# zdzhaoyong/GSLAM

Measured on AMD Instinct MI355X. Metric: orb_extract_plus_bf_match_Mkeypoints_per_s, higher is better.
Workload: dtype u8

## Files before the change

### gslam_amd/csrc/orb.hip

```cpp
#include <stdlib.h>

#include "common.h"
#include "orb_quadtree.h"
#include "../../include/gslam_orb_tables.h"

namespace {

constexpr int kEdge = GH_ORB_EDGE;
constexpr int kCell = GH_ORB_CELL;
constexpr int kCap = GH_ORB_CELL_CAP;
constexpr int kMaxL = GH_ORB_MAX_LEVELS;
constexpr int kHistBins = kCap * 256;
constexpr int kCellRec = 8;

enum {
  kDbgCells = 0,
  kDbgDenseCells,
  kDbgOverflowCells,
  kDbgCapCells,
  kDbgRankDropped,
  kDbgStrongSilenced,
  kDbgMaxQueue,
  kDbgMaxNz,
  kDbgSelCut,
// ... 14 lines not shown
};

__device__ __forceinline__ int xcd_strip_tile(int lin, int total) {
  const int chunk = (total + 7) >> 3;
  return (lin & 7) * chunk + (lin >> 3);
}

__global__ void copy_rows_kernel(const uint8_t* __restrict__ src, size_t src_frame_stride, int src_pitch,
                                 uint8_t* __restrict__ dst, size_t dst_frame_stride, int dst_pitch, int w, int h) {
  int x = blockIdx.x * blockDim.x + threadIdx.x;
  int y = blockIdx.y;
  if (x >= w) return;
  dst[(size_t)blockIdx.z * dst_frame_stride + (size_t)y * dst_pitch + x] =
      src[(size_t)blockIdx.z * src_frame_stride + (size_t)y * src_pitch + x];
}

constexpr int kResizeRows = 4;
constexpr int kResizeCols = 8;

typedef uint32_t u32x4_a4 __attribute__((ext_vector_type(4), aligned(4)));

__device__ __forceinline__ uint32_t mad_u24(uint32_t a, uint32_t b, uint32_t c) {
  uint32_t d;
  asm("v_mad_u32_u24 %0, %1, %2, %3" : "=v"(d) : "v"(a), "v"(b), "v"(c));
  return d;
}

struct ResizeTabs {
  const uint32_t* xtab;
  const uint32_t* xsel;
  const uint32_t* xwgt;
  const uint32_t* ytab;
  const uint32_t* mtab = nullptr;
  const uint32_t* mcw = nullptr;
};

__device__ __forceinline__ void resize_item(const LevelView& src, const uint8_t* __restrict__ s, uint8_t* __restrict__ d,
                                            int dst_pitch, const ResizeTabs& tb, int x8, int y0, int y_end, bool guard_frame) {
  typedef unsigned short u16x2 __attribute__((ext_vector_type(2)));
  const int sx0 = (int)(tb.xtab[x8] >> 16);
  const uint32_t al = (uint32_t)(sx0 & 3);
  const uint32_t d0 = (uint32_t)sx0 & ~3u;
  const uint4 sa = *reinterpret_cast<const uint4*>(tb.xsel + x8), sb = *reinterpret_cast<const uint4*>(tb.xsel + x8 + 4);
  const uint4 wa = *reinterpret_cast<const uint4*>(tb.xwgt + x8), wb = *reinterpret_cast<const uint4*>(tb.xwgt + x8 + 4);
  const uint32_t selp[8] = {sa.x, sa.y, sa.z, sa.w, sb.x, sb.y, sb.z, sb.w};
  const uint32_t wx[8] = {wa.x, wa.y, wa.z, wa.w, wb.x, wb.y, wb.z, wb.w};
  const bool guard = guard_frame && (int)d0 + 16 > src.pitch;
  const uint32_t last_dw = (uint32_t)src.pitch - 4u;
  const uint32_t pitch = (uint32_t)src.pitch;
#pragma unroll
  for (int rr = 0; rr < kResizeRows; ++rr) {
    const int y = y0 + rr;
    if (y >= y_end) break;
    const uint32_t ty = tb.ytab[y];
    const uint32_t sy = ty >> 16;
    const uint32_t fy = ty & 0xFFFFu;
    const uint32_t sy1 = sy + 1 < (uint32_t)src.h ? sy + 1 : (uint32_t)src.h - 1;
    const uint32_t o0 = __umul24(sy, pitch), o1 = __umul24(sy1, pitch);
    u32x4_a4 u, v;
    if (guard && sy1 == (uint32_t)src.h - 1) {
      auto ld = [&](uint32_t row, uint32_t k) { return *reinterpret_cast<const uint32_t*>(s + row + min(d0 + 4u * k, last_dw)); };
      u = u32x4_a4{ld(o0, 0), ld(o0, 1), ld(o0, 2), ld(o0, 3)};
      v = u32x4_a4{ld(o1, 0), ld(o1, 1), ld(o1, 2), ld(o1, 3)};
    } else {
      u = *reinterpret_cast<const u32x4_a4*>(s + (o0 + d0));
      v = *reinterpret_cast<const u32x4_a4*>(s + (o1 + d0));
    }
    const uint32_t uw[3] = {__builtin_amdgcn_alignbyte(u.y, u.x, al), __builtin_amdgcn_alignbyte(u.z, u.y, al),
                            __builtin_amdgcn_alignbyte(u.w, u.z, al)};
    const uint32_t vw[3] = {__builtin_amdgcn_alignbyte(v.y, v.x, al), __builtin_amdgcn_alignbyte(v.z, v.y, al),
                            __builtin_amdgcn_alignbyte(v.w, v.z, al)};
    const uint32_t wy0 = 4u * (2048u - fy), wy1 = 4u * fy;
    uint32_t r[8];
#pragma unroll
    for (int i = 0; i < 8; ++i) {
      const int wsel = i >= 4 ? 1 : 0;
      const u16x2 pu = __builtin_bit_cast(u16x2, __builtin_amdgcn_perm(uw[wsel + 1], uw[wsel], selp[i]));
      const u16x2 pv = __builtin_bit_cast(u16x2, __builtin_amdgcn_perm(vw[wsel + 1], vw[wsel], selp[i]));
      const u16x2 w2 = __builtin_bit_cast(u16x2, wx[i]);
      const uint32_t h0 = __builtin_amdgcn_udot2(pu, w2, 0u, false);
      const uint32_t h1 = __builtin_amdgcn_udot2(pv, w2, 0u, false);
      r[i] = mad_u24(h0, wy0, mad_u24(h1, wy1, 1u << 23));
    }
    uint2 packed;
    packed.x = __builtin_amdgcn_perm(__builtin_amdgcn_perm(r[3], r[2], 0x0c0c0703u), __builtin_amdgcn_perm(r[1], r[0], 0x0c0c0703u), 0x05040100u);
    packed.y = __builtin_amdgcn_perm(__builtin_amdgcn_perm(r[7], r[6], 0x0c0c0703u), __builtin_amdgcn_perm(r[5], r[4], 0x0c0c0703u), 0x05040100u);
    *reinterpret_cast<uint2*>(d + (__umul24((uint32_t)y, (uint32_t)dst_pitch) + (uint32_t)x8)) = packed;
  }
}

__global__ __launch_bounds__(256) void resize_kernel(LevelView src, uint8_t* __restrict__ dst_base,
                                                     size_t dst_frame_stride, int dst_pitch, int wd, int hd,
                                                     ResizeTabs tb, int groups_per_row,
                                                     uint32_t groups_inv, int n_items, int tail_unsafe_frame) {
  const int item = blockIdx.x * 256 + threadIdx.x;
  if (item >= n_items) return;
  const int rg = (int)__umulhi((uint32_t)item, groups_inv);
  const int x8 = (item - rg * groups_per_row) * kResizeCols;
  const int y0 = rg * kResizeRows;
  resize_item(src, src.base + (size_t)blockIdx.y * src.frame_stride, dst_base + (size_t)blockIdx.y * dst_frame_stride, dst_pitch,
              tb, x8, y0, min(hd, y0 + kResizeRows), (int)blockIdx.y == tail_unsafe_frame);
}

struct NextLevel {
  uint8_t* dst_base;
  size_t dst_frame_stride;
  int dst_pitch, hd;
  ResizeTabs tb;
  const int32_t* gx0;
  const int32_t* gy0;
  int tail_unsafe_frame;
  uint32_t tiles_inv = 0, nbx_inv = 0;
  uint8_t* plane = nullptr;
  size_t plane_frame_stride = 0;
  int plane_pitch = 0;
};

inline uint32_t magic_div(uint32_t d, uint32_t n_max) {
  if (d == 0) return 0;
  if (d == 1) return 0;
  const uint64_t inv = ((1ull << 32) + d - 1) / d;
  const uint64_t excess = inv * d - (1ull << 32);
  return (inv < (1ull << 32) && (uint64_t)n_max * excess < (1ull << 32)) ? (uint32_t)inv : 0u;
}

struct ResizeOps {
  uint4 aw[4];
  int cwv[4];
  uint32_t ty;
};
__device__ __forceinline__ ResizeOps resize_tile_mfma_load(int ax, const ResizeTabs& tb, int g0, int ng, int r0, int r1) {
  const int lane = threadIdx.x & 63, n16 = lane & 15;
  const int rb = __builtin_amdgcn_readfirstlane((int)(threadIdx.x >> 6));
  const int ncb = (ng + 1) >> 1;
  const int yq = r0 + 16 * rb + n16, y = yq < r1 ? yq : r1 - 1;
  ResizeOps o;
  o.ty = tb.ytab[y];
#pragma unroll
  for (int cb = 0; cb < 4; ++cb) {
    const int g = g0 + 2 * (cb < ncb ? cb : 0);
    o.aw[cb] = *reinterpret_cast<const uint4*>(tb.mtab + ((size_t)g * 64 + lane) * 4);
    o.cwv[cb] = (int)tb.mcw[g] - ax;
  }
  return o;
}
__device__ __forceinline__ void resize_tile_mfma(const uint8_t* tile, int tile_pitch, int oy, uint8_t* __restrict__ d,
                                                 int dst_pitch, const ResizeOps& ops, int g0, int ng, int r0, int r1,
                                                 uint32_t* __restrict__ dbg) {
  typedef _Float16 f16x8 __attribute__((ext_vector_type(8)));
  typedef float f32x4 __attribute__((ext_vector_type(4)));
  const int lane = threadIdx.x & 63, n16 = lane & 15, q4 = lane >> 4;
  const int rb = __builtin_amdgcn_readfirstlane((int)(threadIdx.x >> 6));
  if (r0 + 16 * rb >= r1) return;
  const int ncb = (ng + 1) >> 1;
  const int yq = r0 + 16 * rb + n16, y = yq < r1 ? yq : r1 - 1;
  const uint32_t ty = ops.ty;
  const uint4 (&aw)[4] = ops.aw;
  const int (&cwv)[4] = ops.cwv;
  const int R = (int)(ty >> 16) - oy;
  const uint32_t fy = ty & 0xFFFFu;
  const uint32_t wy0 = 2048u - fy, wy1 = fy, c23 = 1u << 23, k64 = 0x64646464u;
  const uint8_t* row1 = tile + R * tile_pitch + 8 * q4;
  const uint8_t* row2 = row1 + tile_pitch;
  const uint32_t rowoff = __umul24((uint32_t)y, (uint32_t)dst_pitch);
#pragma unroll
  for (int half = 0; half < 2; ++half) {
    if (2 * half >= ncb) break;
    uint32_t u[2][4], v[2][4];
#pragma unroll
    for (int e = 0; e < 2; ++e) {
      const int cb = 2 * half + e;
      const uint2 b1 = *reinterpret_cast<const uint2*>(row1 + cwv[cb]);
      const uint2 b2 = *reinterpret_cast<const uint2*>(row2 + cwv[cb]);
      uint4 f1, f2;
      f1.x = __builtin_amdgcn_perm(k64, b1.x, 0x04010400u);
// ... 129 lines not shown
  uint32_t a, d;
  __device__ __forceinline__ explicit CompassQ(uint32_t t) : a((((t + 1u) >> 2) + 127u) * 0x01010101u), d((128u - ((t + 1u) >> 2)) * 0x01010101u) {}
};
__device__ __forceinline__ uint32_t fast_compass4_q(const CompassQ& k, uint32_t wc, uint32_t wl, uint32_t wr, uint32_t wu, uint32_t wd) {
  constexpr uint32_t kQ = 0x3F3F3F3Fu;
  const uint32_t c = (wc >> 2) & kQ, u = (wu >> 2) & kQ, d = (wd >> 2) & kQ;
  const uint32_t l = (__builtin_amdgcn_alignbyte(wc, wl, 1) >> 2) & kQ, r = (__builtin_amdgcn_alignbyte(wr, wc, 3) >> 2) & kQ;
  const uint32_t A = c + k.a, Dk = c + k.d;
  const uint32_t not_bright_lr = (A - l) & (A - r);
  const uint32_t bright = __builtin_amdgcn_bitop3_b32(A - u, A - d, not_bright_lr, 0x15);
  const uint32_t dark_lr = (Dk - l) | (Dk - r);
  const uint32_t dark = __builtin_amdgcn_bitop3_b32(Dk - u, Dk - d, dark_lr, 0xA8);
  return bright | dark;
}

#ifndef GH_FAST_WAVES
#define GH_FAST_WAVES 8
#endif
#ifdef GH_ORB_PHASES
__device__ unsigned int* g_orb_phase_buf;
__shared__ unsigned long long ph_t;
__shared__ unsigned int ph_slot;
#define GH_PHASE_START() do { if (threadIdx.x == 0) ph_t = wall_clock64(); } while (0)
#define GH_PHASE(k) do { if (threadIdx.x == 0) { const unsigned long long now_ = wall_clock64(); g_orb_phase_buf[(size_t)ph_slot * 8 + (k)] = (unsigned int)(now_ - ph_t); ph_t = now_; } } while (0)
#else
#define GH_PHASE_START()
#define GH_PHASE(k)
#endif
constexpr int kTileW = 96;
constexpr int kTileH = 72;
constexpr int kScoreH = 66;
constexpr int kScoreOff = 3;

__device__ __forceinline__ void fast_tile_coords(const NextLevel& nx, int nbx, int nby, int tile_id, int& frame, int& bx, int& by) {
  if (nx.tiles_inv != 0u && nx.nbx_inv != 0u) {
    frame = (int)__umulhi((uint32_t)tile_id, nx.tiles_inv);
    const int trem = tile_id - frame * (nbx * nby);
    by = (int)__umulhi((uint32_t)trem, nx.nbx_inv);
    bx = trem - by * nbx;
  } else {
    frame = tile_id / (nbx * nby);
    const int trem = tile_id - frame * (nbx * nby);
    bx = trem % nbx;
    by = trem / nbx;
  }
}
__device__ __forceinline__ const uint4* fast_tile_src(const LevelView& lv, int frame, int bx, int by, int i) {
  const int row = (int)(__umul24((uint32_t)i, 10923u) >> 16), c = i - row * 6;
  int gy = kEdge + 64 * by - 4 + row;
  gy = gy < 0 ? 0 : (gy > lv.h - 1 ? lv.h - 1 : gy);
  int gx = 64 * bx + 16 * c;
  gx = gx > lv.pitch - 16 ? lv.pitch - 16 : gx;
  return reinterpret_cast<const uint4*>(lv.base + (size_t)frame * lv.frame_stride + (__umul24((uint32_t)gy, (uint32_t)lv.pitch) + (uint32_t)gx));
}

constexpr uint32_t kWeakCell = 0xFFFFFFFFu;

__device__ __forceinline__ int hint_threshold(uint32_t word, uint32_t epoch, int ini_th) {
  return ((word >> 16) & 255u) != 0u && (epoch & 1u) != 0u ? ini_th : (int)(word & 255u);
}

template <int PITCH, bool WEAK>
__device__ __forceinline__ int fast_cell_stage(const uint8_t* sc, uint16_t* list2, uint32_t* list, int lane, int ini_th,
                                               uint32_t* __restrict__ rec, uint32_t* __restrict__ ovf,
                                               uint32_t* __restrict__ dbg, int* nz_out) {
  static_assert(PITCH % 4 == 0, "a lane reads its 16 score bytes as dwords");
  const uint64_t lt_mask = (1ull << lane) - 1ull;
  int nz = 0;
  {
    const int row = lane >> 1, cb = 16 * (lane & 1);
    const uint32_t* sp32 = reinterpret_cast<const uint32_t*>(&sc[row * PITCH + cb]);
    uint32_t nzb = 0;
#pragma unroll
    for (int dwi = 0; dwi < 4; ++dwi) {
      const uint32_t w = sp32[dwi];
      const uint32_t f = ((((w & 0x7f7f7f7fu) + 0x7f7f7f7fu) | w) >> 7) & 0x01010101u;
      nzb |= __builtin_amdgcn_udot4(f, 0x08040201u, 0u, false) << (4 * dwi);
    }
    const int cnt = __popc(nzb);
    const int incl = wave_incl_scan_i32(cnt);
// ... 72 lines not shown
        int m2 = 0;
        for (int base = 0; base < n; base += 64) {
          const int i = base + lane;
          const uint32_t e = i < n ? list[i] : 0u;
          const bool keep = i < n && (int)(e >> 10) > ini_th;
          const uint64_t m = __ballot(keep);
          if (keep) list[m2 + __popcll(m & lt_mask)] = e;
          m2 += __popcll(m);
        }
        if (dbg != nullptr && lane == 0 && m2 != n) atomicAdd(&dbg[kDbgStrongSilenced], 1u);
        n = m2;
      }
      if (dbg != nullptr && lane == 0 && !strong && n > 0) atomicAdd(&dbg[kDbgWeakCells], 1u);
    }
    if (dbg != nullptr && lane == 0) {
      atomicAdd(&dbg[kDbgDenseCells], 1u);
      if (n > kCap) atomicAdd(&dbg[kDbgRankDropped], 1u);
    }
    for (int base = 0; base < n; base += 64) {
      const int i = base + lane;
      const uint32_t key = i < n ? list[i] : 0xFFFFFFFFu;
      int rank = 0;
      for (int j = 0; j < n; ++j) rank += list[j] > key ? 1 : 0;
      const bool keep = i < n && rank < kCap;
      const uint64_t m = __ballot(keep);
      if (keep) put_entry(kept + __popcll(m & lt_mask), ((uint32_t)rank << 18) | (key ^ 0x3FFu));
      kept += __popcll(m);
    }
  }
  return kept;
}

template <bool PLANE, bool TWO_PHASE>
__device__ __forceinline__ void fast_cells_tile(const LevelView& lv, int ncx, int ncy, int min_th, int ini_th, bool two,
                                                const uint32_t* __restrict__ hint, int th_a, uint32_t epoch,
                                                uint32_t* __restrict__ cell_cnt, uint32_t* __restrict__ cell_ent,
                                                int cells_per_frame, int cell_off, int n_frames, const NextLevel& nx,
                                                uint32_t* __restrict__ dbg, int tile_id) {
  bool phase_a = TWO_PHASE && two;
  int score_th = min_th;
  constexpr int kScoreW = 68;
  constexpr int kScoreBytes = kScoreH * kScoreW + 8;
  constexpr int kQueueLen = kScoreH * kScoreW;
  __shared__ __attribute__((aligned(16))) uint8_t tile[kTileH * kTileW];
  __shared__ __attribute__((aligned(16))) uint8_t score[kScoreBytes];
  uint32_t(*lists)[256] = reinterpret_cast<uint32_t(*)[256]>(tile);
  static_assert(sizeof(tile) >= 4 * 256 * sizeof(uint32_t), "four 1 KB lists fit the tile");
  __shared__ uint16_t queue[kQueueLen];
  __shared__ int q_count;
  __shared__ uint16_t bit_pos[32];
  GH_PHASE_START();

  const int tid = threadIdx.x;
  __builtin_assume(tid >= 0 && tid < 256);
  const int nbx = (ncx + 1) >> 1, nby = (ncy + 1) >> 1;
  int frame, bx, by;
  fast_tile_coords(nx, nbx, nby, tile_id, frame, bx, by);
  if constexpr (TWO_PHASE) {
    if (phase_a) {
      if (hint != nullptr) th_a = hint_threshold(hint[__builtin_amdgcn_readfirstlane(frame) * kMaxL], epoch, ini_th);
      score_th = th_a;
    }
  }
  const bool pass1_quant = TWO_PHASE && phase_a && th_a > ini_th;
#ifdef GH_ORB_PHASES
  if (threadIdx.x == 0) {
    const unsigned int slot_ = (unsigned int)(frame * cells_per_frame + cell_off + by * nbx + bx);
    ph_slot = slot_;
    g_orb_phase_buf[(size_t)slot_ * 8 + 6] = 1u;
  }
#endif
  static_assert(kTileW / 16 == 6 && kTileH * (kTileW / 16) <= 512 && kTileH * (kTileW / 16) > 256, "two 16-byte items per thread");
  if (tid == 0) q_count = 0;
  const int x0 = kEdge + 64 * bx, y0 = kEdge + 64 * by;
  const int oy = y0 - 4;
  const int ax = 64 * bx;
  const uint8_t* img = lv.base + (size_t)frame * lv.frame_stride;

  bool resized = false;
  ResizeOps rops;
  int rg0 = 0, rng = 0, rr0 = 0, rr1 = 0;
  if (nx.dst_base != nullptr && nx.tb.mtab != nullptr && by > 0 && by < nby - 1 && bx < nbx - 1) {
    rg0 = nx.gx0[bx];
    rng = nx.gx0[bx + 1] - rg0;
    if (rng <= 8) {
      rr0 = nx.gy0[by];
      rr1 = nx.gy0[by + 1];
      rops = resize_tile_mfma_load(ax, nx.tb, rg0, rng, rr0, rr1);
      resized = true;
    }
  }
  for (int i = tid; i < kTileH * (kTileW / 16); i += 256) *reinterpret_cast<uint4*>(&tile[16 * i]) = *fast_tile_src(lv, frame, bx, by, i);
  if (tid < 32) {
    const int ix = tid ^ 15;
    const int k = pass1_quant ? tid >> 3 : (ix & 1) + 2 * (ix >> 4), trip = pass1_quant ? 7 - (tid & 7) : (ix >> 1) & 7;
    bit_pos[tid] = (uint16_t)(1024 * trip + 1 + k);
  }
  __syncthreads();
  GH_PHASE(0);
  if (resized) resize_tile_mfma(tile, kTileW, oy, nx.dst_base + (size_t)frame * nx.dst_frame_stride, nx.dst_pitch, rops, rg0, rng, rr0, rr1, dbg);

  static_assert(kScoreBytes % 16 == 0, "the score tile is cleared by 16-byte stores");
  for (int i = tid; i < kScoreBytes / 16; i += 256) reinterpret_cast<uint4*>(score)[i] = make_uint4(0u, 0u, 0u, 0u);
  const int sx_lo = max(0, kEdge - (x0 - 1)), sx_hi = min(kScoreH, lv.w - kEdge - (x0 - 1));
  const bool interior = sx_lo == 0 && sx_hi == kScoreH && y0 - 1 >= kEdge && y0 - 1 + kScoreH <= lv.h - kEdge;
  constexpr int kItemsPerRow = 17, kItems = kScoreH * kItemsPerRow;
  constexpr int kTrips = (kItems + 255) / 256;
  static_assert(2 * kTrips <= 14 && kScoreW == 4 * kItemsPerRow, "candidate bits of all trips share one dword");
  const uint32_t* tile32 = reinterpret_cast<const uint32_t*>(tile);
  auto pass1 = [&](int th, bool quant) {
    const uint32_t t = (uint32_t)__builtin_amdgcn_readfirstlane(min(max(th, 0), 255));
    const uint32_t tid3856 = (uint32_t)tid * 3856u;
    uint32_t allbits = 0;
    auto trips = [&](auto flags4, int shift, uint32_t mask) {
#pragma unroll
      for (int trip = 0; trip < kTrips; ++trip) {
        const int item = 256 * trip + tid;
        if (item < kItems) {
          const uint32_t sy = (tid3856 + 3856u * 256u * (uint32_t)trip) >> 16;
          const uint32_t ix = (uint32_t)item + 7u * sy + (3 * (kTileW / 4) + 4);
          const uint32_t wc = tile32[ix], wl = tile32[ix - 1], wr = tile32[ix + 1];
          const uint32_t wu = tile32[ix - 3 * (kTileW / 4)], wd = tile32[ix + 3 * (kTileW / 4)];
          const uint32_t w = flags4(wc, wl, wr, wu, wd);
          allbits = __builtin_amdgcn_bitop3_b32(allbits, w >> (shift * trip), mask >> (shift * trip), 0xF8);
        }
      }
    };
    if (quant) {
      const CompassQ cq(t);
      trips([&](uint32_t wc, uint32_t wl, uint32_t wr, uint32_t wu, uint32_t wd) { return fast_compass4_q(cq, wc, wl, wr, wu, wd); }, 1, 0x80808080u);
// ... 68 lines not shown
      if (y0 + r < lv.h && x0 + kQtPlaneX + 4 * cd + 3 < nx.plane_pitch)
        *reinterpret_cast<uint32_t*>(pl + (__umul24((uint32_t)(y0 + r), (uint32_t)nx.plane_pitch) + (uint32_t)(x0 + kQtPlaneX + 4 * cd))) =
            s32[17 * (r + 1) + 1 + cd];
    }
    return;
  }
  const int wv = tid >> 6, lane = tid & 63;
  const int cx = 2 * bx + (wv & 1), cy = 2 * by + (wv >> 1);
  if (cx >= ncx || cy >= ncy) return;
  const uint8_t* sc = &score[(1 + 32 * (wv >> 1)) * kScoreW + kScoreOff + 1 + 32 * (wv & 1)];
  uint16_t* list2 = queue + wv * 1024;
  const size_t cell = (size_t)frame * cells_per_frame + cell_off + (size_t)(__umul24((uint32_t)cy, (uint32_t)ncx) + (uint32_t)cx);
  uint32_t* rec = cell_cnt + cell * kCellRec;
  uint32_t* ovf = cell_ent + cell * kCap;
  int nz, kept;
  if (phase_a) {
    kept = fast_cell_stage<kScoreW, false>(sc, list2, lists[wv], lane, ini_th, rec, ovf, dbg, &nz);
    if (lane == 0) rec[0] = kept == 0 ? kWeakCell : (uint32_t)kept;
  } else {
    kept = fast_cell_stage<kScoreW, true>(sc, list2, lists[wv], lane, ini_th, rec, ovf, dbg, &nz);
    if (lane == 0) rec[0] = (uint32_t)kept;
  }
  GH_PHASE(3);
  if (dbg != nullptr && lane == 0) {
    atomicAdd(&dbg[kDbgCells], 1u);
    if (kept > kCellRec - 1) atomicAdd(&dbg[kDbgOverflowCells], 1u);
    if (kept == kCap) atomicAdd(&dbg[kDbgCapCells], 1u);
    atomicMax(&dbg[kDbgMaxQueue], (uint32_t)nq);
    atomicMax(&dbg[kDbgMaxNz], (uint32_t)nz);
  }
}

template <bool PLANE>
__global__ __launch_bounds__(256, GH_FAST_WAVES) void fast_cells_kernel(LevelView lv, int ncx, int ncy, int min_th, int ini_th,
                                                         uint32_t* __restrict__ cell_cnt,
                                                         uint32_t* __restrict__ cell_ent, int cells_per_frame,
                                                         int cell_off, int n_frames, NextLevel nx,
                                                         uint32_t* __restrict__ dbg, int two_phase,
                                                         const uint32_t* __restrict__ hint, int th_a, uint32_t epoch) {
  const int total = ((ncx + 1) >> 1) * ((ncy + 1) >> 1) * n_frames;
  const int tile_id = xcd_strip_tile(blockIdx.x, total);
  if (tile_id >= total) return;
  fast_cells_tile<PLANE, !PLANE>(lv, ncx, ncy, min_th, ini_th, two_phase != 0, hint, th_a, epoch, cell_cnt, cell_ent, cells_per_frame, cell_off,
                                 n_frames, nx, dbg, tile_id);
}

struct AllLevels {
  LevelView lv[kMaxL];
  int ncx[kMaxL], ncy[kMaxL], cell_off[kMaxL], tile_start[kMaxL + 1];
  int n_levels;
};
__global__ __launch_bounds__(256) void fast_cells_all_kernel(AllLevels A, int min_th, int ini_th,
                                                             uint32_t* __restrict__ cell_cnt,
                                                             uint32_t* __restrict__ cell_ent, int cells_per_frame,
                                                             int n_frames, uint32_t* __restrict__ dbg) {
  int l = 0;
  for (int k = 1; k < A.n_levels; ++k)
    if ((int)blockIdx.x >= A.tile_start[k]) l = k;
  const NextLevel none{nullptr, 0, 0, 0, ResizeTabs{nullptr, nullptr, nullptr, nullptr}, nullptr, nullptr, -1};
  fast_cells_tile<false, false>(A.lv[l], A.ncx[l], A.ncy[l], min_th, ini_th, false, nullptr, ini_th, 0u, cell_cnt, cell_ent, cells_per_frame, A.cell_off[l],
                                n_frames, none, dbg, (int)blockIdx.x - A.tile_start[l]);
}

__device__ __forceinline__ int block_excl_scan(int v, int* wave_tot , int* total) {
  const int lane = threadIdx.x & 63, wv = threadIdx.x >> 6;
  int incl = v;
#pragma unroll
  for (int o = 1; o < 64; o <<= 1) {
    int t = __shfl_up(incl, o);
    if (lane >= o) incl += t;
  }
  __syncthreads();
  if (lane == 63) wave_tot[wv] = incl;
  __syncthreads();
  int off = 0;
  for (int k = 0; k < wv; ++k) off += wave_tot[k];
  *total = wave_tot[0] + wave_tot[1] + wave_tot[2] + wave_tot[3];
  return off + incl - v;
}

template <typename F>
__device__ __forceinline__ void for_each_overflow(const uint32_t* __restrict__ ovf, int n, F f) {
  static_assert(kCellRec - 1 == 7 && kCap % 4 == 0, "entry 8 starts the 16-byte groups");
  if (n > 7) f(ovf[7]);
  for (int e = 8; e < n; e += 4) {
    const uint4 w = *reinterpret_cast<const uint4*>(ovf + e);
    f(w.x);
    if (e + 1 < n) f(w.y);
    if (e + 2 < n) f(w.z);
    if (e + 3 < n) f(w.w);
  }
}

__device__ __forceinline__ int cell_entries(uint32_t count) { return count <= (uint32_t)kCap ? (int)count : 0; }
// ... 787 lines not shown
  long long r = 1;
  while (e-- > 0) r *= b;
  return r;
}

}

extern "C" uint32_t gh_magic_div(uint32_t d, uint32_t n_max) { return magic_div(d, n_max); }

struct gh_orb_plan {
  gh_ctx* ctx = nullptr;
  int w = 0, h = 0, max_batch = 0, L = 0;
  gh_orb_params prm{};
  int lw[kMaxL]{}, lh[kMaxL]{}, pitch[kMaxL]{}, quota[kMaxL]{}, quota_off[kMaxL]{};
  int ncx[kMaxL]{}, ncy[kMaxL]{}, cell_off[kMaxL]{};
  float scale[kMaxL]{};
  size_t lvl_off[kMaxL]{};
  size_t slab = 0;
  int cells_per_frame = 0;
  int max_level_cells = 0;
  uint8_t* pyr = nullptr;
  uint32_t* xtab[kMaxL]{};
  uint32_t* ytab[kMaxL]{};
  uint32_t* xsel[kMaxL]{};
  uint32_t* xwgt[kMaxL]{};
  uint32_t* mtab[kMaxL]{};
  uint32_t* mcw[kMaxL]{};
  uint32_t* cell_cnt = nullptr;
  uint32_t* cell_ent = nullptr;
  SelKp* sel = nullptr;
  int32_t* level_cnt = nullptr;
  const int32_t* own_gx[kMaxL] = {nullptr};
  const int32_t* own_gy[kMaxL] = {nullptr};
  int8_t* d_pattern = nullptr;
  int8_t* d_base_pattern = nullptr;
  int8_t base_pattern[256 * 4] = {};
  bool base_pattern_fits_table = true;
  int distribution = 0;
  gh_qt_plan* qt = nullptr;
  uint8_t* score_plane = nullptr;
  size_t plane_off[kMaxL] = {}, plane_slab = 0;
  int plane_pitch[kMaxL] = {};
  int steer = 0;
  int32_t* d_dir = nullptr;
  uint32_t* tabs = nullptr;
  uint32_t* dbg = nullptr;
  bool dbg_on = false;
  uint32_t* hint = nullptr;
  int hint_mode = GH_ORB_HINT_ADAPTIVE, hint_value = 0;
  uint32_t hint_epoch = kHintFirstEpoch;
  struct CallGraph {
    const void *gray, *kps, *desc, *counts;
    int batch, row_stride;
    size_t frame_stride;
    hipGraphExec_t exec;
    hipEvent_t done;
  };
  static constexpr int kGraphRing = 16, kGraphGiveUp = 8;
  std::vector<CallGraph> graphs, retired;
  long long graph_hits = 0, graph_misses = 0;
  hipStream_t cap_stream = nullptr;
  bool graphs_off = false;
  hipStream_t side = nullptr;
  hipEvent_t ev_level[kMaxL]{}, ev_join = nullptr;
  uint8_t* stage_img = nullptr;
  uint8_t* stage_out = nullptr;
// ... 167 lines not shown
      long long num = (long long)K * ipow(5, l) * ipow(6, L - 1 - l);
      p->quota[l] = (int)((2 * num + den) / (2 * den));
      if (p->quota[l] > K - qsum) p->quota[l] = K - qsum;
      qsum += p->quota[l];
    } else {
      p->quota[l] = K - qsum > 0 ? K - qsum : 0;
    }
    p->scale[l] = l == 0 ? 1.0f : p->scale[l - 1] * 1.2f;
    const int vw = p->lw[l] - 2 * kEdge, vh = p->lh[l] - 2 * kEdge;
    p->ncx[l] = vw > 0 ? (vw + kCell - 1) / kCell : 0;
    p->ncy[l] = vh > 0 ? (vh + kCell - 1) / kCell : 0;
    if (p->ncx[l] == 0 || p->ncy[l] == 0) p->ncx[l] = p->ncy[l] = 0;
    p->cell_off[l] = coff;
    coff += p->ncx[l] * p->ncy[l];
    if (p->ncx[l] * p->ncy[l] > p->max_level_cells) p->max_level_cells = p->ncx[l] * p->ncy[l];
  }
  int qo = 0;
  for (int l = 0; l < L; ++l) {
    p->quota_off[l] = qo;
    qo += p->quota[l];
  }
  p->slab = off + 256;
  p->cells_per_frame = coff > 0 ? coff : 1;
}

static size_t pad8(size_t n) { return (n + 7) & ~(size_t)7; }
static size_t axis_words(int n_dst) { return pad8((size_t)n_dst); }
static size_t lerp_words(int wd) { return 2 * pad8((size_t)wd); }
static size_t mfma_words(int wd) {
  const size_t ngr = ((size_t)wd + 7) / 8;
  return ngr * 256 + pad8(ngr);
}
static size_t own_words(int ncells) { return pad8((size_t)(ncells + 1) / 2 + 1); }

static size_t plan_table_words(const gh_orb_plan* p) {
  size_t words = 0;
  for (int l = 1; l < p->L; ++l) words += axis_words(p->lw[l]) + lerp_words(p->lw[l]) + axis_words(p->lh[l]);
  for (int l = 1; l < p->L; ++l) words += mfma_words(p->lw[l]);
  for (int l = 0; l + 1 < p->L; ++l) words += own_words(p->ncx[l]) + own_words(p->ncy[l]);
  return words;
}

static gh_status plan_allocate(gh_orb_plan* p, size_t tab_words) {
  const size_t B = (size_t)p->max_batch;
  const int K = p->prm.n_features;
  GH_TRY(plan_alloc(p, B * p->slab, (void**)&p->pyr));
  GH_TRY(plan_alloc(p, B * p->cells_per_frame * kCellRec * sizeof(uint32_t), (void**)&p->cell_cnt));
  GH_TRY(plan_alloc(p, B * p->cells_per_frame * kCap * sizeof(uint32_t), (void**)&p->cell_ent));
  GH_TRY(plan_alloc(p, B * K * sizeof(SelKp), (void**)&p->sel));
  GH_TRY(plan_alloc(p, B * kMaxL * sizeof(int32_t), (void**)&p->level_cnt));
  GH_TRY(plan_alloc(p, sizeof(GH_ORB_PATTERN), (void**)&p->d_pattern));
  GH_TRY(plan_alloc(p, 256 * 4, (void**)&p->d_base_pattern));
  GH_TRY(plan_alloc(p, sizeof(GH_ORB_DIR), (void**)&p->d_dir));
  GH_TRY(plan_alloc(p, (B * kMaxL + 2) * sizeof(uint32_t), (void**)&p->hint));
  return plan_alloc(p, tab_words * sizeof(uint32_t), (void**)&p->tabs);
}

static void build_axis_table(std::vector<uint32_t>& htab, size_t& tw, int n_src, int n_dst, bool x_axis) {
  for (int x = 0; x < n_dst; ++x) {
    long long P = ((long long)(2 * x + 1) * n_src * 2048) / (2LL * n_dst) - 1024;
    if (P < 0) P = 0;
    int sx = (int)(P >> 11), fx = (int)(P & 2047);
    if (sx >= n_src - 1) {
      sx = n_src - 1;
      fx = 0;
    }
    htab[tw++] = ((uint32_t)sx << 16) | (uint32_t)fx;
  }
  while (tw & 7) {
    htab[tw] = x_axis ? ((htab[tw - 1] >> 16) + 1u) << 16 : htab[tw - 1];
    ++tw;
  }
// ... 55 lines not shown
      for (int e = 0; e < 4; ++e) mt[((size_t)g * 64 + lane) * 4 + e] = wds[e];
    }
  }
  p->mtab[l] = ok ? p->tabs + tw : nullptr;
  p->mcw[l] = ok ? p->tabs + tw + (size_t)ngr * 256 : nullptr;
  tw += mfma_words(wd);
}

static void build_own_tables(gh_orb_plan* p, int l, std::vector<uint32_t>& htab, size_t& tw) {
  const int nbx = (p->ncx[l] + 1) / 2, nby = (p->ncy[l] + 1) / 2;
  const uint32_t* xt = htab.data() + (p->xtab[l + 1] - p->tabs);
  const uint32_t* yt = htab.data() + (p->ytab[l + 1] - p->tabs);
  const int ngroups = (p->lw[l + 1] + 7) / 8, hd = p->lh[l + 1];
  p->own_gx[l] = reinterpret_cast<const int32_t*>(p->tabs + tw);
  int g = 0;
  for (int bx = 0; bx <= nbx; ++bx) {
    if (bx == nbx) g = ngroups;
    else
      while (bx > 0 && g < ngroups && (int)(xt[8 * g] >> 16) < 64 * bx) ++g;
    htab[tw++] = (uint32_t)g;
  }
  while (tw & 7) htab[tw++] = (uint32_t)ngroups;
  p->own_gy[l] = reinterpret_cast<const int32_t*>(p->tabs + tw);
  int y = 0;
  for (int by = 0; by <= nby; ++by) {
    if (by == nby) y = hd;
    else
      while (by > 0 && y < hd && (int)(yt[y] >> 16) < 64 * by + 15) ++y;
    htab[tw++] = (uint32_t)y;
  }
  while (tw & 7) htab[tw++] = (uint32_t)hd;
}

static gh_status plan_build_tables(gh_orb_plan* p, std::vector<uint32_t>& htab, size_t tab_words) {
  const int L = p->L;
  size_t tw = 0;
  for (int l = 1; l < L; ++l) {
    p->xtab[l] = p->tabs + tw;
    build_axis_table(htab, tw, p->lw[l - 1], p->lw[l], true);
    const size_t nx_pad = axis_words(p->lw[l]);
    p->xsel[l] = p->tabs + tw;
    p->xwgt[l] = p->tabs + tw + nx_pad;
    if (!build_lerp_tables(htab, tw, tw - nx_pad, nx_pad, p->lw[l - 1]))
      return gh_set_error(p->ctx, GH_ERR_ARG, "resize table violates the 8-column window contract (level size ratio is not ~1.2)");
    p->ytab[l] = p->tabs + tw;
    build_axis_table(htab, tw, p->lh[l - 1], p->lh[l], false);
  }
  for (int l = 1; l < L; ++l) build_mfma_tables(p, l, htab, tw);
  for (int l = 0; l + 1 < L; ++l) build_own_tables(p, l, htab, tw);
  if (tw != tab_words) return gh_set_error(p->ctx, GH_ERR_ARG, "gh_orb_plan_create: the tables take %zu words, %zu were planned", tw, tab_words);
  return GH_OK;
}

static gh_status plan_upload(gh_orb_plan* p, const std::vector<uint32_t>& htab) {
  gh_ctx* ctx = p->ctx;
  GH_TRY(gh_dev_upload(ctx, p->tabs, htab.data(), htab.size() * sizeof(uint32_t)));
  GH_TRY(upload_pattern(p, &GH_ORB_PATTERN[0][0][0]));
  memcpy(p->base_pattern, &GH_ORB_PATTERN[0][0][0], sizeof(p->base_pattern));
  GH_TRY(gh_dev_upload(ctx, p->d_base_pattern, p->base_pattern, sizeof(p->base_pattern)));
  GH_HIP(ctx, hipMemsetD32Async((hipDeviceptr_t)p->hint, p->prm.ini_th_fast, (size_t)p->max_batch * kMaxL + 2, ctx->stream));
  return gh_dev_upload(ctx, p->d_dir, GH_ORB_DIR, sizeof(GH_ORB_DIR));
}

static gh_status plan_init(gh_orb_plan* p) {
  plan_geometry(p);
  const size_t tab_words = plan_table_words(p);
  std::vector<uint32_t> htab(tab_words ? tab_words : 1);
  GH_TRY(plan_allocate(p, htab.size()));
  GH_TRY(plan_build_tables(p, htab, tab_words));
  return plan_upload(p, htab);
}

extern "C" gh_status gh_orb_plan_create(gh_ctx* ctx, int width, int height, int max_batch,
                                        const gh_orb_params* params, gh_orb_plan** out) {
  if (!ctx || !out) return GH_ERR_ARG;
  GH_ENTER(ctx);
  *out = nullptr;
  gh_orb_params prm;
  gh_orb_default_params(&prm);
  if (params) prm = *params;
  GH_TRY(plan_check_params(ctx, width, height, max_batch, prm));
  GH_HIP(ctx, hipSetDevice(ctx->device));
// ... 142 lines not shown

static SelectArgs select_args(const gh_orb_plan* p) {
  SelectArgs sa;
  for (int l = 0; l < kMaxL; ++l) {
    sa.ncells[l] = l < p->L ? p->ncx[l] * p->ncy[l] : 0;
    sa.cell_off[l] = l < p->L ? p->cell_off[l] : 0;
    sa.ncx[l] = l < p->L && p->ncx[l] > 0 ? p->ncx[l] : 1;
    sa.quota[l] = l < p->L ? p->quota[l] : 0;
    sa.quota_off[l] = l < p->L ? p->quota_off[l] : 0;
  }
  return sa;
}

static gh_status launch_select(const OrbCall& c, const SelectArgs& sa, int l0, int nl) {
  const gh_orb_plan* p = c.p;
  gh_ctx* ctx = p->ctx;
  SelectWeak weak;
  for (int l = 0; l < kMaxL; ++l) weak.lv[l] = c.lv[l < p->L ? l : 0];
  weak.min_th = p->prm.min_th_fast;
  weak.ini_th = p->prm.ini_th_fast;
  weak.two_phase = c.s.two_phase ? 1 : 0;
  uint32_t* const hints = c.s.hint_adaptive ? p->hint : nullptr;
  if (c.s.sel_cached)
    GH_LAUNCH(ctx, "orb_select", select_kernel<true>, dim3(nl, c.batch), dim3(256), 0, sa, p->cell_cnt, p->cell_ent,
              p->cells_per_frame, p->prm.n_features, p->sel, p->level_cnt, c.dbg, l0, weak, hints, c.s.th_a,
              p->hint + (size_t)p->max_batch * kMaxL, c.s.hint_epoch);
  else
    GH_LAUNCH(ctx, "orb_select", select_kernel<false>, dim3(nl, c.batch), dim3(256), 0, sa, p->cell_cnt, p->cell_ent,
              p->cells_per_frame, p->prm.n_features, p->sel, p->level_cnt, c.dbg, l0, weak, hints, c.s.th_a,
              p->hint + (size_t)p->max_batch * kMaxL, c.s.hint_epoch);
  return GH_OK;
}

static NextLevel next_level_args(const OrbCall& c, int l, long long tiles) {
  const gh_orb_plan* p = c.p;
  NextLevel nx{nullptr, 0, 0, 0, ResizeTabs{nullptr, nullptr, nullptr, nullptr}, nullptr, nullptr, -1};
  if (l + 1 < p->L)
    nx = NextLevel{p->pyr + p->lvl_off[l + 1], p->slab, p->pitch[l + 1], p->lh[l + 1],
                   ResizeTabs{p->xtab[l + 1], p->xsel[l + 1], p->xwgt[l + 1], p->ytab[l + 1], p->mtab[l + 1], p->mcw[l + 1]},
                   p->own_gx[l], p->own_gy[l], (l == 0 && c.s.zero_copy0) ? c.batch - 1 : -1};
  const uint32_t nbx = (uint32_t)gh_div_up(p->ncx[l], 2), tpf = nbx * (uint32_t)gh_div_up(p->ncy[l], 2);
  nx.tiles_inv = magic_div(tpf, (uint32_t)tiles);
  nx.nbx_inv = magic_div(nbx, tpf);
  return nx;
}

static gh_status fast_level(const OrbCall& c, int l, bool plane) {
  const gh_orb_plan* p = c.p;
  gh_ctx* ctx = p->ctx;
  const long long tiles = (long long)gh_div_up(p->ncx[l], 2) * gh_div_up(p->ncy[l], 2) * c.batch;
  GH_CHECK_ARG(ctx, tiles < (1LL << 30));
  NextLevel nx = next_level_args(c, l, tiles);
  const dim3 grid(8 * gh_div_up(tiles, 8));
  if (plane) {
    nx.plane = p->score_plane + p->plane_off[l];
    nx.plane_frame_stride = p->plane_slab;
    nx.plane_pitch = p->plane_pitch[l];
    GH_LAUNCH(ctx, "orb_fast_plane", fast_cells_kernel<true>, grid, dim3(256), 0, c.lv[l], p->ncx[l], p->ncy[l], p->prm.min_th_fast,
              p->prm.ini_th_fast, p->cell_cnt, p->cell_ent, p->cells_per_frame, p->cell_off[l], c.batch, nx, c.dbg, 0, nullptr, 0, 0u);
  } else {
    GH_LAUNCH(ctx, "orb_fast_cells", fast_cells_kernel<false>, grid, dim3(256), 0, c.lv[l], p->ncx[l], p->ncy[l], p->prm.min_th_fast,
              p->prm.ini_th_fast, p->cell_cnt, p->cell_ent, p->cells_per_frame, p->cell_off[l], c.batch, nx, c.dbg, c.s.two_phase ? 1 : 0,
              c.s.hint_adaptive ? p->hint + l : nullptr, c.s.th_a, c.s.hint_epoch);
  }
  return GH_OK;
}

static gh_status enqueue_quadtree(const OrbCall& c) {
  const gh_orb_plan* p = c.p;
  gh_ctx* ctx = p->ctx;
  GH_TRY(gh_qt_begin(ctx, p->qt, c.batch));
  for (int l = 0; l < p->L; ++l) {
    if (p->ncx[l] == 0 || !gh_qt_plane_ok(p->qt, l)) {
      GH_TRY(gh_qt_cells(ctx, p->qt, l, c.lv[l], nullptr, c.batch, p->prm.min_th_fast, p->prm.ini_th_fast));
      if (l + 1 < p->L) GH_TRY(resize_standalone(c, l + 1));
      continue;
    }
    GH_TRY(fast_level(c, l, true));
    const LevelView plane{p->score_plane + p->plane_off[l], p->plane_slab, p->plane_pitch[l], p->lw[l], p->lh[l]};
    GH_TRY(gh_qt_cells(ctx, p->qt, l, c.lv[l], &plane, c.batch, p->prm.min_th_fast, p->prm.ini_th_fast));
  }
  return gh_qt_tree(ctx, p->qt, c.batch, p->quota_off, p->prm.n_features, p->sel, p->level_cnt);
}

static AllLevels all_levels_args(const OrbCall& c, int* tiles_out) {
  const gh_orb_plan* p = c.p;
  const int L = p->L;
  AllLevels A;
  A.n_levels = L;
  int tiles = 0;
  for (int l = 0; l < kMaxL; ++l) {
    A.tile_start[l] = tiles;
    A.lv[l] = c.lv[l < L ? l : 0];
    A.ncx[l] = l < L ? p->ncx[l] : 0;
    A.ncy[l] = l < L ? p->ncy[l] : 0;
    A.cell_off[l] = l < L ? p->cell_off[l] : 0;
// ... 327 lines not shown
```

Before: 230.5.

## Precompute per-tile resize records and issue tile loads before dependent setup

Adds host-built per-tile column and row records holding the group start, group count, column offsets and row range, so the FAST tile kernel fetches them with one aligned load each. This replaces the chained gx0/gy0/mcw lookups. Kernel arguments are repacked into a leading TileHead struct and pinned to scalar registers. The tile's global loads and the hint word are now issued at kernel entry, ahead of the dependent setup, so their latency overlaps that work. The resize path also reads four ytab entries with a single vector load. The cost is extra table memory, plus risk in the more complex argument layout and the alignment assumption on ytab.

```diff
diff --git a/gslam_amd/csrc/orb.hip b/gslam_amd/csrc/orb.hip
--- a/gslam_amd/csrc/orb.hip
+++ b/gslam_amd/csrc/orb.hip
@@ -70,7 +70,6 @@
   const uint32_t* xwgt;
   const uint32_t* ytab;
   const uint32_t* mtab = nullptr;
-  const uint32_t* mcw = nullptr;
 };
 
 __device__ __forceinline__ void resize_item(const LevelView& src, const uint8_t* __restrict__ s, uint8_t* __restrict__ d,
@@ -86,11 +85,12 @@
   const bool guard = guard_frame && (int)d0 + 16 > src.pitch;
   const uint32_t last_dw = (uint32_t)src.pitch - 4u;
   const uint32_t pitch = (uint32_t)src.pitch;
+  const u32x4_a4 ty4 = *reinterpret_cast<const u32x4_a4*>(tb.ytab + y0);
 #pragma unroll
   for (int rr = 0; rr < kResizeRows; ++rr) {
     const int y = y0 + rr;
     if (y >= y_end) break;
-    const uint32_t ty = tb.ytab[y];
+    const uint32_t ty = ty4[rr];
     const uint32_t sy = ty >> 16;
     const uint32_t fy = ty & 0xFFFFu;
     const uint32_t sy1 = sy + 1 < (uint32_t)src.h ? sy + 1 : (uint32_t)src.h - 1;
@@ -148,11 +148,29 @@
   const int32_t* gx0;
   const int32_t* gy0;
   int tail_unsafe_frame;
-  uint32_t tiles_inv = 0, nbx_inv = 0;
   uint8_t* plane = nullptr;
   size_t plane_frame_stride = 0;
   int plane_pitch = 0;
 };
+
+struct alignas(32) TileColRec {
+  int g0, ng;
+  int cw[4];
+  int pad[2];
+};
+struct alignas(8) TileRowRec {
+  int r0, r1;
+};
+static_assert(sizeof(TileColRec) == 32 && sizeof(TileRowRec) == 8, "one aligned scalar load per record");
+
+struct TileHead {
+  const uint8_t* base;
+  size_t frame_stride;
+  int pitch, w, h;
+  int ncx, ncy, n_frames;
+  uint32_t tiles_inv, nbx_inv;
+};
+static_assert(sizeof(TileHead) == 48, "with the two pointers behind it: the 64 leading argument bytes");
 
 inline uint32_t magic_div(uint32_t d, uint32_t n_max) {
   if (d == 0) return 0;
@@ -167,18 +185,18 @@
   int cwv[4];
   uint32_t ty;
 };
-__device__ __forceinline__ ResizeOps resize_tile_mfma_load(int ax, const ResizeTabs& tb, int g0, int ng, int r0, int r1) {
+__device__ __forceinline__ ResizeOps resize_tile_mfma_load(const ResizeTabs& tb, const TileColRec& c, int r0, int r1) {
   const int lane = threadIdx.x & 63, n16 = lane & 15;
   const int rb = __builtin_amdgcn_readfirstlane((int)(threadIdx.x >> 6));
-  const int ncb = (ng + 1) >> 1;
+  const int ncb = (c.ng + 1) >> 1;
   const int yq = r0 + 16 * rb + n16, y = yq < r1 ? yq : r1 - 1;
   ResizeOps o;
   o.ty = tb.ytab[y];
 #pragma unroll
   for (int cb = 0; cb < 4; ++cb) {
-    const int g = g0 + 2 * (cb < ncb ? cb : 0);
+    const int g = c.g0 + 2 * (cb < ncb ? cb : 0);
     o.aw[cb] = *reinterpret_cast<const uint4*>(tb.mtab + ((size_t)g * 64 + lane) * 4);
-    o.cwv[cb] = (int)tb.mcw[g] - ax;
+    o.cwv[cb] = c.cw[cb];
   }
   return o;
 }
@@ -374,11 +392,11 @@
 constexpr int kScoreH = 66;
 constexpr int kScoreOff = 3;
 
-__device__ __forceinline__ void fast_tile_coords(const NextLevel& nx, int nbx, int nby, int tile_id, int& frame, int& bx, int& by) {
-  if (nx.tiles_inv != 0u && nx.nbx_inv != 0u) {
-    frame = (int)__umulhi((uint32_t)tile_id, nx.tiles_inv);
+__device__ __forceinline__ void fast_tile_coords(const TileHead& hd, int nbx, int nby, int tile_id, int& frame, int& bx, int& by) {
+  if (hd.tiles_inv != 0u && hd.nbx_inv != 0u) {
+    frame = (int)__umulhi((uint32_t)tile_id, hd.tiles_inv);
     const int trem = tile_id - frame * (nbx * nby);
-    by = (int)__umulhi((uint32_t)trem, nx.nbx_inv);
+    by = (int)__umulhi((uint32_t)trem, hd.nbx_inv);
     bx = trem - by * nbx;
   } else {
     frame = tile_id / (nbx * nby);
@@ -387,7 +405,7 @@
     by = trem / nbx;
   }
 }
-__device__ __forceinline__ const uint4* fast_tile_src(const LevelView& lv, int frame, int bx, int by, int i) {
+__device__ __forceinline__ const uint4* fast_tile_src(const TileHead& lv, int frame, int bx, int by, int i) {
   const int row = (int)(__umul24((uint32_t)i, 10923u) >> 16), c = i - row * 6;
   int gy = kEdge + 64 * by - 4 + row;
   gy = gy < 0 ? 0 : (gy > lv.h - 1 ? lv.h - 1 : gy);
@@ -526,11 +544,13 @@
 }
 
 template <bool PLANE, bool TWO_PHASE>
-__device__ __forceinline__ void fast_cells_tile(const LevelView& lv, int ncx, int ncy, int min_th, int ini_th, bool two,
-                                                const uint32_t* __restrict__ hint, int th_a, uint32_t epoch,
+__device__ __forceinline__ void fast_cells_tile(const TileHead& hd, const uint32_t* __restrict__ hint,
+                                                const TileColRec* __restrict__ tile_rec, int min_th, int ini_th, bool two, int th_a, uint32_t epoch,
                                                 uint32_t* __restrict__ cell_cnt, uint32_t* __restrict__ cell_ent,
-                                                int cells_per_frame, int cell_off, int n_frames, const NextLevel& nx,
+                                                int cells_per_frame, int cell_off, const NextLevel& nx,
                                                 uint32_t* __restrict__ dbg, int tile_id) {
+  const LevelView lv{hd.base, hd.frame_stride, hd.pitch, hd.w, hd.h};
+  const int ncx = hd.ncx, ncy = hd.ncy;
   bool phase_a = TWO_PHASE && two;
   int score_th = min_th;
   constexpr int kScoreW = 68;
@@ -549,10 +569,27 @@
   __builtin_assume(tid >= 0 && tid < 256);
   const int nbx = (ncx + 1) >> 1, nby = (ncy + 1) >> 1;
   int frame, bx, by;
-  fast_tile_coords(nx, nbx, nby, tile_id, frame, bx, by);
+  fast_tile_coords(hd, nbx, nby, tile_id, frame, bx, by);
+  constexpr int kTileItems = kTileH * (kTileW / 16);
+  static_assert(kTileW / 16 == 6 && kTileItems <= 512 && kTileItems > 256, "two 16-byte items per thread");
+  const uint4 item0 = *fast_tile_src(hd, frame, bx, by, tid);
+  const uint4 item1 = *fast_tile_src(hd, frame, bx, by, min(tid + 256, kTileItems - 1));
+  uint32_t hint_word = 0u;
+  if constexpr (TWO_PHASE) {
+    if (hint != nullptr) hint_word = hint[frame * kMaxL];
+  }
+  TileColRec crec{};
+  TileRowRec rrec{};
+  const bool has_rec = tile_rec != nullptr && by > 0 && by < nby - 1 && bx < nbx - 1;
+  if (has_rec) {
+    crec = tile_rec[bx];
+    rrec = reinterpret_cast<const TileRowRec*>(tile_rec + nbx)[by];
+  }
+  int rng = crec.ng;
+  asm("" : "+s"(rng) : "s"(min_th), "s"(ini_th), "s"((int)two), "s"(th_a), "s"(epoch));
   if constexpr (TWO_PHASE) {
     if (phase_a) {
-      if (hint != nullptr) th_a = hint_threshold(hint[__builtin_amdgcn_readfirstlane(frame) * kMaxL], epoch, ini_th);
+      if (hint != nullptr) th_a = hint_threshold(hint_word, epoch, ini_th);
       score_th = th_a;
     }
   }
@@ -564,32 +601,21 @@
     g_orb_phase_buf[(size_t)slot_ * 8 + 6] = 1u;
   }
 #endif
-  static_assert(kTileW / 16 == 6 && kTileH * (kTileW / 16) <= 512 && kTileH * (kTileW / 16) > 256, "two 16-byte items per thread");
   if (tid == 0) q_count = 0;
   const int x0 = kEdge + 64 * bx, y0 = kEdge + 64 * by;
   const int oy = y0 - 4;
-  const int ax = 64 * bx;
-  const uint8_t* img = lv.base + (size_t)frame * lv.frame_stride;
-
-  bool resized = false;
+
+  const bool resized = has_rec && rng <= 8;
   ResizeOps rops;
-  int rg0 = 0, rng = 0, rr0 = 0, rr1 = 0;
-  if (nx.dst_base != nullptr && nx.tb.mtab != nullptr && by > 0 && by < nby - 1 && bx < nbx - 1) {
-    rg0 = nx.gx0[bx];
-    rng = nx.gx0[bx + 1] - rg0;
-    if (rng <= 8) {
-      rr0 = nx.gy0[by];
-      rr1 = nx.gy0[by + 1];
-      rops = resize_tile_mfma_load(ax, nx.tb, rg0, rng, rr0, rr1);
-      resized = true;
-    }
-  }
-  for (int i = tid; i < kTileH * (kTileW / 16); i += 256) *reinterpret_cast<uint4*>(&tile[16 * i]) = *fast_tile_src(lv, frame, bx, by, i);
+  const int rg0 = crec.g0, rr0 = rrec.r0, rr1 = rrec.r1;
+  if (resized) rops = resize_tile_mfma_load(nx.tb, crec, rr0, rr1);
   if (tid < 32) {
     const int ix = tid ^ 15;
     const int k = pass1_quant ? tid >> 3 : (ix & 1) + 2 * (ix >> 4), trip = pass1_quant ? 7 - (tid & 7) : (ix >> 1) & 7;
     bit_pos[tid] = (uint16_t)(1024 * trip + 1 + k);
   }
+  *reinterpret_cast<uint4*>(&tile[16 * tid]) = item0;
+  if (tid + 256 < kTileItems) *reinterpret_cast<uint4*>(&tile[16 * (tid + 256)]) = item1;
   __syncthreads();
   GH_PHASE(0);
   if (resized) resize_tile_mfma(tile, kTileW, oy, nx.dst_base + (size_t)frame * nx.dst_frame_stride, nx.dst_pitch, rops, rg0, rng, rr0, rr1, dbg);
@@ -724,17 +750,19 @@
 }
 
 template <bool PLANE>
-__global__ __launch_bounds__(256, GH_FAST_WAVES) void fast_cells_kernel(LevelView lv, int ncx, int ncy, int min_th, int ini_th,
+__global__ __launch_bounds__(256, GH_FAST_WAVES) void fast_cells_kernel(TileHead hd, const uint32_t* __restrict__ hint,
+                                                         const TileColRec* __restrict__ tile_rec, int min_th, int ini_th,
                                                          uint32_t* __restrict__ cell_cnt,
                                                          uint32_t* __restrict__ cell_ent, int cells_per_frame,
-                                                         int cell_off, int n_frames, NextLevel nx,
-                                                         uint32_t* __restrict__ dbg, int two_phase,
-                                                         const uint32_t* __restrict__ hint, int th_a, uint32_t epoch) {
-  const int total = ((ncx + 1) >> 1) * ((ncy + 1) >> 1) * n_frames;
+                                                         int cell_off, NextLevel nx,
+                                                         uint32_t* __restrict__ dbg, int two_phase, int th_a, uint32_t epoch) {
+  int ncx = hd.ncx;
+  asm("" : "+s"(ncx) : "s"(hd.base), "s"(hd.frame_stride), "s"(hd.pitch), "s"(hd.w), "s"(hd.h), "s"(hd.ncy), "s"(hd.n_frames),
+                        "s"(hd.tiles_inv), "s"(hd.nbx_inv), "s"(hint), "s"(tile_rec));
+  const int total = ((ncx + 1) >> 1) * ((hd.ncy + 1) >> 1) * hd.n_frames;
   const int tile_id = xcd_strip_tile(blockIdx.x, total);
   if (tile_id >= total) return;
-  fast_cells_tile<PLANE, !PLANE>(lv, ncx, ncy, min_th, ini_th, two_phase != 0, hint, th_a, epoch, cell_cnt, cell_ent, cells_per_frame, cell_off,
-                                 n_frames, nx, dbg, tile_id);
+  fast_cells_tile<PLANE, !PLANE>(hd, hint, tile_rec, min_th, ini_th, two_phase != 0, th_a, epoch, cell_cnt, cell_ent, cells_per_frame, cell_off, nx, dbg, tile_id);
 }
 
 struct AllLevels {
@@ -750,8 +778,10 @@
   for (int k = 1; k < A.n_levels; ++k)
     if ((int)blockIdx.x >= A.tile_start[k]) l = k;
   const NextLevel none{nullptr, 0, 0, 0, ResizeTabs{nullptr, nullptr, nullptr, nullptr}, nullptr, nullptr, -1};
-  fast_cells_tile<false, false>(A.lv[l], A.ncx[l], A.ncy[l], min_th, ini_th, false, nullptr, ini_th, 0u, cell_cnt, cell_ent, cells_per_frame, A.cell_off[l],
-                                n_frames, none, dbg, (int)blockIdx.x - A.tile_start[l]);
+  const LevelView& lv = A.lv[l];
+  const TileHead hd{lv.base, lv.frame_stride, lv.pitch, lv.w, lv.h, A.ncx[l], A.ncy[l], n_frames, 0u, 0u};
+  fast_cells_tile<false, false>(hd, nullptr, nullptr, min_th, ini_th, false, ini_th, 0u, cell_cnt, cell_ent, cells_per_frame, A.cell_off[l], none, dbg,
+                                (int)blockIdx.x - A.tile_start[l]);
 }
 
 __device__ __forceinline__ int block_excl_scan(int v, int* wave_tot , int* total) {
@@ -1605,6 +1635,7 @@
   int32_t* level_cnt = nullptr;
   const int32_t* own_gx[kMaxL] = {nullptr};
   const int32_t* own_gy[kMaxL] = {nullptr};
+  const TileColRec* tile_rec[kMaxL] = {nullptr};
   int8_t* d_pattern = nullptr;
   int8_t* d_base_pattern = nullptr;
   int8_t base_pattern[256 * 4] = {};
@@ -1838,12 +1869,14 @@
   return ngr * 256 + pad8(ngr);
 }
 static size_t own_words(int ncells) { return pad8((size_t)(ncells + 1) / 2 + 1); }
+static size_t tile_rec_words(int ncx, int ncy) { return 8 * (size_t)((ncx + 1) / 2) + pad8(2 * (size_t)((ncy + 1) / 2)); }
 
 static size_t plan_table_words(const gh_orb_plan* p) {
   size_t words = 0;
   for (int l = 1; l < p->L; ++l) words += axis_words(p->lw[l]) + lerp_words(p->lw[l]) + axis_words(p->lh[l]);
   for (int l = 1; l < p->L; ++l) words += mfma_words(p->lw[l]);
   for (int l = 0; l + 1 < p->L; ++l) words += own_words(p->ncx[l]) + own_words(p->ncy[l]);
+  for (int l = 0; l + 1 < p->L; ++l) words += tile_rec_words(p->ncx[l], p->ncy[l]);
   return words;
 }
 
@@ -1965,6 +1998,32 @@
   while (tw & 7) htab[tw++] = (uint32_t)hd;
 }
 
+static void build_tile_records(gh_orb_plan* p, int l, std::vector<uint32_t>& htab, size_t& tw) {
+  const int nbx = (p->ncx[l] + 1) / 2, nby = (p->ncy[l] + 1) / 2;
+  const size_t words = tile_rec_words(p->ncx[l], p->ncy[l]);
+  const bool ok = p->mcw[l + 1] != nullptr;
+  if (ok) {
+    const uint32_t* gx = htab.data() + (reinterpret_cast<const uint32_t*>(p->own_gx[l]) - p->tabs);
+    const uint32_t* gy = htab.data() + (reinterpret_cast<const uint32_t*>(p->own_gy[l]) - p->tabs);
+    const uint32_t* mc = htab.data() + (p->mcw[l + 1] - p->tabs);
+    for (int bx = 0; bx < nbx; ++bx) {
+      const int g0 = (int)gx[bx], ng = (int)gx[bx + 1] - g0, ncb = (ng + 1) / 2;
+      uint32_t* r = htab.data() + tw + 8 * (size_t)bx;
+      r[0] = (uint32_t)g0;
+      r[1] = (uint32_t)ng;
+      for (int cb = 0; cb < 4; ++cb)
+        r[2 + cb] = ng >= 1 && ng <= 8 ? (uint32_t)((int)mc[g0 + 2 * (cb < ncb ? cb : 0)] - 64 * bx) : 0u;
+      r[6] = r[7] = 0u;
+    }
+    for (int by = 0; by < nby; ++by) {
+      htab[tw + 8 * (size_t)nbx + 2 * (size_t)by] = gy[by];
+      htab[tw + 8 * (size_t)nbx + 2 * (size_t)by + 1] = gy[by + 1];
+    }
+  }
+  p->tile_rec[l] = ok ? reinterpret_cast<const TileColRec*>(p->tabs + tw) : nullptr;
+  tw += words;
+}
+
 static gh_status plan_build_tables(gh_orb_plan* p, std::vector<uint32_t>& htab, size_t tab_words) {
   const int L = p->L;
   size_t tw = 0;
@@ -1981,6 +2040,7 @@
   }
   for (int l = 1; l < L; ++l) build_mfma_tables(p, l, htab, tw);
   for (int l = 0; l + 1 < L; ++l) build_own_tables(p, l, htab, tw);
+  for (int l = 0; l + 1 < L; ++l) build_tile_records(p, l, htab, tw);
   if (tw != tab_words) return gh_set_error(p->ctx, GH_ERR_ARG, "gh_orb_plan_create: the tables take %zu words, %zu were planned", tw, tab_words);
   return GH_OK;
 }
@@ -2189,17 +2249,22 @@
   return GH_OK;
 }
 
-static NextLevel next_level_args(const OrbCall& c, int l, long long tiles) {
+static NextLevel next_level_args(const OrbCall& c, int l) {
   const gh_orb_plan* p = c.p;
   NextLevel nx{nullptr, 0, 0, 0, ResizeTabs{nullptr, nullptr, nullptr, nullptr}, nullptr, nullptr, -1};
   if (l + 1 < p->L)
     nx = NextLevel{p->pyr + p->lvl_off[l + 1], p->slab, p->pitch[l + 1], p->lh[l + 1],
-                   ResizeTabs{p->xtab[l + 1], p->xsel[l + 1], p->xwgt[l + 1], p->ytab[l + 1], p->mtab[l + 1], p->mcw[l + 1]},
+                   ResizeTabs{p->xtab[l + 1], p->xsel[l + 1], p->xwgt[l + 1], p->ytab[l + 1], p->mtab[l + 1]},
                    p->own_gx[l], p->own_gy[l], (l == 0 && c.s.zero_copy0) ? c.batch - 1 : -1};
+  return nx;
+}
+
+static TileHead tile_head_args(const OrbCall& c, int l, long long tiles) {
+  const gh_orb_plan* p = c.p;
+  const LevelView& lv = c.lv[l];
   const uint32_t nbx = (uint32_t)gh_div_up(p->ncx[l], 2), tpf = nbx * (uint32_t)gh_div_up(p->ncy[l], 2);
-  nx.tiles_inv = magic_div(tpf, (uint32_t)tiles);
-  nx.nbx_inv = magic_div(nbx, tpf);
-  return nx;
+  return TileHead{lv.base, lv.frame_stride, lv.pitch, lv.w, lv.h, p->ncx[l], p->ncy[l], c.batch,
+                  magic_div(tpf, (uint32_t)tiles), magic_div(nbx, tpf)};
 }
 
 static gh_status fast_level(const OrbCall& c, int l, bool plane) {
@@ -2207,18 +2272,20 @@
   gh_ctx* ctx = p->ctx;
   const long long tiles = (long long)gh_div_up(p->ncx[l], 2) * gh_div_up(p->ncy[l], 2) * c.batch;
   GH_CHECK_ARG(ctx, tiles < (1LL << 30));
-  NextLevel nx = next_level_args(c, l, tiles);
+  NextLevel nx = next_level_args(c, l);
   const dim3 grid(8 * gh_div_up(tiles, 8));
+  const TileColRec* trec = l + 1 < p->L ? p->tile_rec[l] : nullptr;
   if (plane) {
     nx.plane = p->score_plane + p->plane_off[l];
     nx.plane_frame_stride = p->plane_slab;
     nx.plane_pitch = p->plane_pitch[l];
-    GH_LAUNCH(ctx, "orb_fast_plane", fast_cells_kernel<true>, grid, dim3(256), 0, c.lv[l], p->ncx[l], p->ncy[l], p->prm.min_th_fast,
-              p->prm.ini_th_fast, p->cell_cnt, p->cell_ent, p->cells_per_frame, p->cell_off[l], c.batch, nx, c.dbg, 0, nullptr, 0, 0u);
+    GH_LAUNCH(ctx, "orb_fast_plane", fast_cells_kernel<true>, grid, dim3(256), 0, tile_head_args(c, l, tiles), nullptr, trec, p->prm.min_th_fast,
+              p->prm.ini_th_fast, p->cell_cnt, p->cell_ent, p->cells_per_frame, p->cell_off[l], nx, c.dbg, 0, 0, 0u);
   } else {
-    GH_LAUNCH(ctx, "orb_fast_cells", fast_cells_kernel<false>, grid, dim3(256), 0, c.lv[l], p->ncx[l], p->ncy[l], p->prm.min_th_fast,
-              p->prm.ini_th_fast, p->cell_cnt, p->cell_ent, p->cells_per_frame, p->cell_off[l], c.batch, nx, c.dbg, c.s.two_phase ? 1 : 0,
-              c.s.hint_adaptive ? p->hint + l : nullptr, c.s.th_a, c.s.hint_epoch);
+    GH_LAUNCH(ctx, "orb_fast_cells", fast_cells_kernel<false>, grid, dim3(256), 0,
+              tile_head_args(c, l, tiles), c.s.hint_adaptive ? p->hint + l : nullptr, trec, p->prm.min_th_fast,
+              p->prm.ini_th_fast, p->cell_cnt, p->cell_ent, p->cells_per_frame, p->cell_off[l], nx, c.dbg, c.s.two_phase ? 1 : 0,
+              c.s.th_a, c.s.hint_epoch);
   }
   return GH_OK;
 }
```

After: 235.6, median of 6. 2.2% higher.
